# Russoul/cuda-mat

Hardware: AMD Instinct MI355X
Metric: BiCGSTAB iters/sec + SpMV effective HBM GB/s, 10M-row CSR at 1/2/4/8 GPUs (higher is better)
Workload: dtype f64

## Files before the change

### cuda_mat_amd/csrc/device.h

```cpp
#pragma once
#include <hip/hip_runtime.h>

#include "batch.h"
#include "kernels.h"
#include "steps.h"

namespace cm {

__device__ __forceinline__ double wave_sum(double v)
{
#pragma unroll
    for (int o = 32; o > 0; o >>= 1) v += __shfl_xor(v, o, 64);
    return v;
}

template <int L>
__device__ __forceinline__ double group_sum(double v)
{
#pragma unroll
    for (int o = L / 2; o > 0; o >>= 1) v += __shfl_xor(v, o, 64);
    return v;
}

template <int K>
__device__ __forceinline__ void block_sum(double (&v)[K], double *lds)
{
    const int wave = threadIdx.x >> 6, lane = threadIdx.x & 63;
#pragma unroll
    for (int k = 0; k < K; k++) v[k] = wave_sum(v[k]);
    __syncthreads();
    if (lane == 0) {
#pragma unroll
        for (int k = 0; k < K; k++) lds[wave * K + k] = v[k];
    }
    __syncthreads();
#pragma unroll
    for (int k = 0; k < K; k++)
        v[k] = ((lds[0 * K + k] + lds[1 * K + k]) + lds[2 * K + k]) + lds[3 * K + k];
}

constexpr int kLongRow = 4096;
constexpr int kLongRowSlots = 32;

struct LongRows {
    int rows[kLongRowSlots];
    int noted;
    int count;
    int next;
};

__device__ __forceinline__ void long_rows_note(LongRows &t, int row)
{
    const int slot = atomicAdd(&t.noted, 1);
    if (slot < kLongRowSlots) t.rows[slot] = row;
}

__device__ __forceinline__ int long_rows_round(LongRows &t, const int *rp, int row_begin, int row_end, int done)
{
    const int total = t.noted;
    if (done >= total) return 0;
    if (threadIdx.x == 0) {
        if (total <= kLongRowSlots) {
            for (int i = 1; i < total; i++) {
                const int r = t.rows[i];
                int j = i - 1;
                while (j >= 0 && t.rows[j] > r) { t.rows[j + 1] = t.rows[j]; j--; }
                t.rows[j + 1] = r;
            }
            t.count = total;
        } else {
            int r = done == 0 ? row_begin : t.next, m = 0;
            for (; r < row_end && m < kLongRowSlots; r++)
                if (rp[r + 1] - rp[r] > kLongRow) t.rows[m++] = r;
            t.count = m;
            t.next = r;
        }
    }
    __syncthreads();
    return t.count;
}

template <int K>
__device__ __forceinline__ void load_scalars(const ScalarSrc &s, double (&out)[K], double *lds)
{
    if (s.count == 0) {
#pragma unroll
        for (int k = 0; k < K; k++) out[k] = s.ptr[k];
        return;
    }
#pragma unroll
    for (int k = 0; k < K; k++) out[k] = 0.0;
    for (int j = threadIdx.x; j < s.count; j += kBlock) {
#pragma unroll
        for (int k = 0; k < K; k++) out[k] += s.ptr[(size_t)j * s.stride + k];
    }
    block_sum<K>(out, lds);
}

__device__ __forceinline__ bool leader() { return blockIdx.x == 0 && threadIdx.x == 0; }

__device__ __forceinline__ int uniform_state(const LoopState *st)
{
    __shared__ int s_state;
    if (threadIdx.x == 0) s_state = st->state;
    __syncthreads();
    const int v = s_state;
    __syncthreads();
    return v;
}

__device__ __forceinline__ void publish_progress(const LoopArgs &la, int state)
{
    if (la.snap && leader())
        __hip_atomic_store(&la.snap[la.k % la.snap_slots],
                           ((unsigned long long)(unsigned)(la.k + 1) << 32) | (unsigned long long)(unsigned)state,
                           __ATOMIC_RELAXED, __HIP_MEMORY_SCOPE_SYSTEM);
}

constexpr double kTolabsMin = 0x1p-485;

__device__ __forceinline__ bool init_refusal(double nrm0, double tolabs, bool r_nonzero)
{
    return !isfinite(nrm0) || (nrm0 == 0.0 && r_nonzero) || (tolabs > 0.0 && tolabs < kTolabsMin);
}

__device__ __forceinline__ bool check_half(const LoopArgs &la, const ScalarSrc &half, double *lds)
{
    LoopState *st = la.st;
    if (uniform_state(st) != 0) return true;
    double sc[1];
    load_scalars<1>(half, sc, lds);
    const double nrm = sqrt(sc[0]);
    const int it = st->it;
    if (la.loop == CUDAMAT_LOOP_PBICGSTAB) {
        if (leader()) {
            st->nrm = nrm;
            if (la.hist && 2 * it < la.hist_cap) la.hist[2 * it] = nrm;
        }
        if (!la.no_exit && nrm < st->tolabs) {
            if (leader()) st->state = 1;
            return true;
        }
        if (!la.no_exit && isnan(nrm)) {
            if (leader()) st->state = 3;
            return true;
        }
    }
    return false;
}

__device__ __forceinline__ bool check_full(const LoopArgs &la, const double (&sc)[2])
{
    LoopState *st = la.st;
    const int it = st->it;
    if (it == 0) return false;
    const double nrm = sqrt(sc[1]);
    const double omega = st->omega;
    if (leader()) {
        st->nrm = nrm;
        if (la.hist) {
            const int slot = (la.loop != CUDAMAT_LOOP_PBICGSTAB2) ? 2 * (it - 1) + 1 : it - 1;
            if (slot < la.hist_cap) la.hist[slot] = nrm;
        }
    }
    if (la.no_exit) return false;
    if (nrm < st->tolabs) {
        if (leader()) st->state = 2;
        return true;
    }
    if (la.loop == CUDAMAT_LOOP_PBICGSTAB2 && (fabs(omega) < 1e-5 || isnan(omega))) {
        if (leader()) st->state = 3;
        return true;
    }
    if (isnan(nrm)) {
        if (leader()) st->state = 3;
        return true;
    }
    return false;
}

template <int K>
__device__ __forceinline__ void load_row(const double *p, int64_t i, double (&v)[K])
{
    if constexpr (K == 1) {
        v[0] = p[i];
    } else {
        const double2 *q = (const double2 *)(p + (size_t)i * K);
#pragma unroll
        for (int h = 0; h < K / 2; h++) {
            const double2 t = q[h];
            v[2 * h] = t.x;
            v[2 * h + 1] = t.y;
        }
    }
}

template <int K>
__device__ __forceinline__ void store_row(double *p, int64_t i, const double (&v)[K], unsigned mask)
{
    if constexpr (K == 1) {
        if (mask & 1u) p[i] = v[0];
    } else {
        double *row = p + (size_t)i * K;
#pragma unroll
        for (int h = 0; h < K / 2; h++) {
            const unsigned m = (mask >> (2 * h)) & 3u;
            if (m == 3u) ((double2 *)row)[h] = make_double2(v[2 * h], v[2 * h + 1]);
            else if (m == 1u) row[2 * h] = v[2 * h];
            else if (m == 2u) row[2 * h + 1] = v[2 * h + 1];
        }
    }
}

constexpr unsigned kAll = 0xffu;
// ... 143 lines not shown
```

### cuda_mat_amd/csrc/loops.hip

```cpp
#include <utility>
#include <math.h>
#include <stdlib.h>
#include <string.h>

#include "solver.h"

using namespace cm;

namespace cm {

int wait_progress(cudamat_solver *s, hipStream_t st, int j, const char *what, unsigned long long *word)
{
    volatile unsigned long long *slot = &s->snap_host[j % kRing];
    unsigned long long w = *slot;
    if ((unsigned)(w >> 32) != (unsigned)(j + 1)) {
        const double t_wait = now_s();
        while ((unsigned)((w = *slot) >> 32) != (unsigned)(j + 1)) {
            __builtin_ia32_pause();
            if (now_s() - t_wait > 30.0) {
                const double t_drain = now_s();
                while (hipStreamQuery(st) == hipErrorNotReady && now_s() - t_drain < 5.0) __builtin_ia32_pause();
                set_error("%siteration %d did not report progress within 30 s%s", what, j,
                          s->sharded ? " (sharded run: this rank must exit, its peers are waiting in a collective)" : "");
                return CUDAMAT_ERR_HIP;
// ... 67 lines not shown
    int pipe_rr = kPipeRR;
    ScalarSrc pipeB_src{nullptr, 0, 1};
    hipStream_t rst = nullptr;

    void prof_mark() { if (profile && hipEventRecord(prof_event(s, pe++), st) != hipSuccess) s->prof_failed = true; }

    int setup();
    int pipelined_prologue();
    bool wants_fused() const;
    bool wants_resident();
    int run_resident(bool *gave_up);
    int run_host_loop();
    int iterate_reference();
    int iterate_fused();
    int iterate_pipelined(int k);
    int pipe_reduce(ScalarSrc parts, int K, double *out, int slot);
    int pipe_wait(int slot);
    int finish(bool *precond_gave_up, cudamat_stats *out);
};

int Solve::setup()
{
    CM_ARG(s && b && x, "null pointer");
    CM_ARG(precond == CUDAMAT_PRECOND_NONE || precond == CUDAMAT_PRECOND_ILU0 || precond == CUDAMAT_PRECOND_BLOCK_ILU0,
           "precond");
    CM_ARG(loop == CUDAMAT_LOOP_PBICGSTAB || loop == CUDAMAT_LOOP_PBICGSTAB2 || loop == CUDAMAT_LOOP_PIPELINED, "loop");
    CM_ARG(maxit >= 0, "maxit");
    CM_ARG(!(precond == CUDAMAT_PRECOND_ILU0 && s->sharded),
           "ILU(0) of the whole matrix is single-GPU only (SURVEY 8e); sharded runs take CUDAMAT_PRECOND_BLOCK_ILU0");
    CM_ARG(!(precond && s->d), "the (A0 + I d) variant has no preconditioner (pbicgstab.h:110)");
    CM_HIP(hipSetDevice(s->ctx->device));
    cfg = &s->ctx->cfg;
    t_begin = now_s();
    st = s->ctx->stream;
    n = s->n;
    x_user = x;
    {
        int rc_setup = ensure_work(s);
        const bool defer_form = s->spmv_mode < 0 && precond == CUDAMAT_PRECOND_ILU0 && !s->sharded;
        if (rc_setup == CUDAMAT_OK && !defer_form) rc_setup = ensure_spmv_mode(s);
        if (rc_setup == CUDAMAT_OK && precond && (!s->has_ilu || (s->sharded && !s->ilu_block)))
            rc_setup = ilu0_setup(s, precond == CUDAMAT_PRECOND_BLOCK_ILU0);
        CM_TRY(setup_agree(s, rc_setup));
    }
    perm = precond == CUDAMAT_PRECOND_ILU0 && !s->sharded && loop == CUDAMAT_LOOP_PBICGSTAB && s->L.lm && s->U.lm && !s->d &&
           cfg->trsv_perm && !s->perm_failed;
    if (perm && !s->perm_ready) {
        const int rcp = ilu_perm_matrix(s);
        if (rcp == CUDAMAT_ERR_NOMEM) { perm = false; s->perm_failed = true; }
        else CM_TRY(rcp);
    }
    s->perm_active = perm;
    if (!perm && s->spmv_mode < 0) CM_TRY(ensure_spmv_mode(s));
    if (perm) {
        CM_TRY(perm_to_space(s, false, b, s->b_perm));
        if (!(flags & CUDAMAT_FLAG_X0_ONES)) CM_TRY(perm_to_space(s, true, x, s->x_perm));
        b = s->b_perm;
        x = s->x_perm;
    }

    const int need_hist = history_need(loop, maxit);
    hist_base = abs_tol > 0.0 ? (s->hist_count < s->hist_cap ? s->hist_count : s->hist_cap) : 0;
    if (hist_base == 0 && need_hist > s->hist_cap) {
        if (s->hist) { CM_HIP(hipStreamSynchronize(st)); CM_DROP(hipFree(s->hist)); s->hist = nullptr; }
        CM_TRY(dev_alloc((void **)&s->hist, sizeof(double) * (size_t)need_hist));
        s->hist_cap = need_hist;
    }
    if (s->hist_cap > hist_base)
        CM_HIP(hipMemsetAsync(s->hist + hist_base, 0xFF, sizeof(double) * (size_t)(s->hist_cap - hist_base), st));
    s->last_loop = loop;
    profile = (flags & CUDAMAT_FLAG_PROFILE) != 0;
    sharded = s->sharded;
    pipelined = loop == CUDAMAT_LOOP_PIPELINED;
    pipe_pc = pipelined && precond != CUDAMAT_PRECOND_NONE;
    la = LoopArgs{s->st, s->hist + hist_base, s->hist_cap - hist_base, loop, (flags & CUDAMAT_FLAG_NO_EXIT) ? 1 : 0, s->snap_dev, kRing, 0};
    for (int i = 0; i < kRing; i++) s->snap_host[i] = 0ULL;

    s->comm_used = 0;
    s->comm_kind.clear();
    s->profiling = profile && sharded;
    s->prof_failed = false;
    t_loop0 = now_s();
    if (flags & CUDAMAT_FLAG_X0_ONES) CM_TRY(launch_fill(st, n, 1.0, x));
    CM_HIP(hipMemcpyAsync(s->pw, x, sizeof(double) * (size_t)n, hipMemcpyDeviceToDevice, st));
    CM_TRY(spmv_local(s, s->pw, s->r, 0, nullptr, nullptr, la_none, CHECK_NONE, nosrc));
    CM_TRY(launch_init(st, n, b, s->r, s->rw, s->p, s->parts_full, &np_full));
    full_src = ScalarSrc{s->parts_full, np_full, 2};
    if (sharded) {
        CM_TRY(launch_reduce_parts(st, full_src, 2, s->red + 4, 0));
        CM_TRY(allreduce(s, s->red + 4, 2));
        full_src = ScalarSrc{s->red + 4, 0, 1};
    }
    CM_TRY(launch_init_finish(st, s->st, full_src, tol, abs_tol, la.no_exit, sharded ? nullptr : s->r, n));
    return CUDAMAT_OK;
}

int Solve::pipelined_prologue()
{
    pipe_rr = cfg->pipe_rr >= 0 ? cfg->pipe_rr : kPipeRR;
    const size_t nb = sizeof(double) * (size_t)(s->n_pad > 0 ? s->n_pad : 1);
    if (!s->pz) {
        double **vs[] = {&s->pz, &s->pww, &s->pq, &s->py, &s->pxh};
        for (double **q : vs) {
            CM_TRY(dev_alloc((void **)q, nb));
            CM_HIP(hipMemsetAsync(*q, 0, nb, st));
        }
        CM_TRY(dev_alloc((void **)&s->pipeA, sizeof(double) * 3 * kVecGridMax));
        CM_TRY(dev_alloc((void **)&s->pipeB, sizeof(double) * 5 * kVecGridMax));
        CM_TRY(dev_alloc((void **)&s->red_pipe, sizeof(double) * 16));
    }
    if (pipe_pc && !s->prh) {
        double **vs[] = {&s->prh, &s->pwh, &s->psh, &s->pzh, &s->pqh, &s->ptmp};
        for (double **q : vs) {
            CM_TRY(dev_alloc((void **)q, nb));
            CM_HIP(hipMemsetAsync(*q, 0, nb, st));
        }
    }
    if (sharded && s->comm.allreduce_side && s->comm.reduce_stream) {
        rst = (hipStream_t)s->comm.reduce_stream;
        for (int e = 0; e < 2; e++) {
            if (!s->ev_red[e]) CM_HIP(hipEventCreateWithFlags(&s->ev_red[e], hipEventDisableTiming));
            if (!s->ev_red_done[e]) CM_HIP(hipEventCreateWithFlags(&s->ev_red_done[e], hipEventDisableTiming));
        }
    }
    const LoopArgs la_freeze{s->st, nullptr, 0, loop, 0};
    const double *rh0 = s->r;
    if (pipe_pc) { CM_TRY(precond_apply(s, s->r, s->ptmp, s->prh)); rh0 = s->prh; }
    CM_TRY(spmv_local(s, rh0, s->pww, 1, s->rw, s->parts_rv, la_freeze, CHECK_NONE, nosrc));
    ScalarSrc rww{s->parts_rv, spmv_parts(s), 2};
    if (sharded) {
        CM_TRY(launch_reduce_parts(st, rww, 1, s->red + 0, 0));
        CM_TRY(allreduce(s, s->red + 0, 1));
        rww = ScalarSrc{s->red + 0, 0, 1};
    }
    const double *wh0 = s->pww;
    if (pipe_pc) { CM_TRY(precond_apply(s, s->pww, s->ptmp, s->pwh)); wh0 = s->pwh; }
    CM_TRY(spmv_local(s, wh0, s->t, 0, nullptr, nullptr, la_freeze, CHECK_NONE, nosrc));
    CM_TRY(launch_pipe_seed(st, full_src, rww, s->red_pipe + 8));
    pipeB_src = ScalarSrc{s->red_pipe + 8, 0, 1};
    return CUDAMAT_OK;
}

int Solve::pipe_reduce(ScalarSrc parts, int K, double *out, int slot)
{
    if (!sharded) return CUDAMAT_OK;
    if (rst) {
        CM_HIP(hipEventRecord(s->ev_red[slot], st));
        CM_HIP(hipStreamWaitEvent(rst, s->ev_red[slot], 0));
        CM_TRY(launch_reduce_parts(rst, parts, K, out, 0));
        comm_mark_begin(s, 3, rst);
        if (s->comm.allreduce_side(s->comm.user, out, K) != 0) { set_error("allreduce_side callback failed"); return CUDAMAT_ERR_COMM; }
        comm_mark_end(s, rst);
        CM_HIP(hipEventRecord(s->ev_red_done[slot], rst));
    } else {
        CM_TRY(launch_reduce_parts(st, parts, K, out, 0));
        CM_TRY(allreduce(s, out, K));
    }
    return CUDAMAT_OK;
}

int Solve::pipe_wait(int slot)
{
    if (sharded && rst) CM_HIP(hipStreamWaitEvent(st, s->ev_red_done[slot], 0));
    return CUDAMAT_OK;
}

int Solve::iterate_pipelined(int k)
{
// ... 431 lines not shown
```

### cuda_mat_amd/csrc/solver.h

```cpp
#pragma once
#include <vector>

#include "kernels.h"
#include "spmv_pb.h"
#include "valdict.h"
#include "spmv_sell.h"
#include "spmv_pat.h"

namespace cm {

constexpr int kLag = 2;
constexpr int kRing = kLag + 2;
constexpr int kPipeRR = 32;

struct TriFactor {
    int nlevels = 0;
    std::vector<int> level_ptr;
    int *rp = nullptr;
    int *ci = nullptr;
    double *val = nullptr;
    int *row_of = nullptr;
    double *dinv = nullptr;
    int64_t nnz = 0;
    int *rhs_of = nullptr, *out_of = nullptr;
// ... 47 lines not shown
    double *v2 = nullptr;
    double *pz = nullptr, *pww = nullptr, *pq = nullptr, *py = nullptr, *pxh = nullptr;
    double *prh = nullptr, *pwh = nullptr, *psh = nullptr, *pzh = nullptr, *pqh = nullptr, *ptmp = nullptr;
    double *pipeA = nullptr, *pipeB = nullptr, *red_pipe = nullptr;
    hipEvent_t ev_red[2] = {}, ev_red_done[2] = {};

    double *parts_full = nullptr, *parts_rv = nullptr, *parts_half = nullptr, *parts_tt = nullptr;
    double *red = nullptr;
    cm::LoopState *st = nullptr;
    cm::LoopState *st_ring = nullptr;
    hipEvent_t ev[cm::kRing] = {};
    unsigned long long *snap_host = nullptr;
    unsigned long long *snap_dev = nullptr;
    double *hist = nullptr;
    int hist_cap = 0;
    int hist_count = 0;
    int last_loop = 0;

    std::vector<hipEvent_t> prof_ev;
    std::vector<hipEvent_t> comm_ev;
    std::vector<int> comm_kind;
    size_t comm_used = 0;
    bool profiling = false;
    bool prof_failed = false;

    bool sharded = false;
    cudamat_comm comm{};
    bool overlap = false;
    bool agreed = false;
    int overlap_chunks = 4;
    hipEvent_t ev_x = nullptr, ev_part[cm::kPbMaxChunks] = {};
    hipStream_t part_stream[cm::kPbMaxChunks] = {};
    hipEvent_t ev_p1[cm::kPbMaxChunks] = {};
    double ms_spmv_alone = 0.0;
    bool windowed = false;
    bool windows_known = false;
    std::vector<int64_t> w_send_off, w_send_cnt, w_recv_off, w_recv_cnt;
    double gather_fraction = 1.0;
    double *need_dev = nullptr;

    bool has_ilu = false;
    int *pm_rp = nullptr, *pm_ci = nullptr;
    double *pm_val = nullptr;
    int64_t pm_nnz = 0;
    bool pm_owned = false;
    bool ilu_block = false;
    double *lu = nullptr;
    int *diag_pos = nullptr;
    cm::TriFactor L, U;
    void *ilu_plans = nullptr;
    cm::PbPlan pb_perm{};
    cm::ValDict vd_perm;
    double *x_perm = nullptr, *b_perm = nullptr;
    bool perm_ready = false;
    bool perm_failed = false;
    bool perm_active = false;
    double t_perm_matrix = 0.0;
    double t_analysis = 0.0, t_factor = 0.0, t_analysis_l = 0.0, t_analysis_u = 0.0;
    int trsv_fallbacks = 0;
    cm::ValDict vd;
    bool vd_tried = false;
    unsigned *bar = nullptr;
    int test_allreduces = 0;
    bool resident_off = false;
    int device_cus = 0;
    int loop_fallbacks = 0;

    cm::ManyWork many;
};

namespace cm {
int dev_alloc(void **p, size_t bytes);
int solver_alloc(cudamat_ctx *ctx, int n_local, int64_t n_cols, int64_t nnz, cudamat_solver **out);
int solver_setup_pattern(cudamat_solver *s);
int solver_setup_values(cudamat_solver *s);
int spmv_mode_is_blocked_early(cudamat_solver *s, bool *blocked);
void spmv_mode_adopt_blocked(cudamat_solver *s, const PbPlan &pb, double seconds);
int ensure_valdict(cudamat_solver *s);
int ensure_work(cudamat_solver *s);
int ensure_spmv_mode(cudamat_solver *s);
int setup_agree(cudamat_solver *s, int rc_local);
int spmv_local(cudamat_solver *s, const double *x_local, double *y, int dot, const double *w, double *parts, LoopArgs la, int check,
               ScalarSrc half);
int spmv_parts(const cudamat_solver *s);
int allreduce(cudamat_solver *s, double *buf, int count);
void comm_mark_begin(cudamat_solver *s, int kind, hipStream_t st);
void comm_mark_end(cudamat_solver *s, hipStream_t st);
hipEvent_t prof_event(cudamat_solver *s, size_t i);
int precond_apply(cudamat_solver *s, const double *in, double *tmp, double *out, bool native = false);

constexpr int kSortRowMax = 1024;
int launch_sort_rows(hipStream_t st, int nrows, const int *src_rp, const int *src_of, const int *dst_rp, const int *ci,
                     const double *val, const int *colmap, int *out_ci, double *out_val);
int ilu0_setup(cudamat_solver *s, bool block);
int ilu0_analyse_early(cudamat_solver *s);
void ilu0_flush_deferred(cudamat_solver *s);
bool ilu0_will_use_level_major(cudamat_solver *s);
int ilu0_release(cudamat_solver *s);
int trsv_apply(cudamat_solver *s, const TriFactor &F, bool upper, const double *rhs, double *out);
int precond_apply_original(cudamat_solver *s, const double *in, double *tmp, double *out);
int perm_to_space(cudamat_solver *s, bool upper, const double *in, double *out);
int perm_from_space(cudamat_solver *s, bool upper, const double *in, double *out);
int ilu_perm_matrix(cudamat_solver *s);
int trsv_status(cudamat_solver *s);
bool trsv_syncfree_active(cudamat_solver *s);
int trsv_form_code(cudamat_solver *s);
void trsv_group_counts(cudamat_solver *s, int *groups_l, int *groups_u);
void trsv_disable_syncfree(cudamat_solver *s);
void many_release(cudamat_solver *s);
int wait_progress(cudamat_solver *s, hipStream_t st, int j, const char *what, unsigned long long *word);
int history_need(int loop, int maxit);
int history_count(int loop, const LoopState &f, int cap);
void stats_from_state(const LoopState &f, cudamat_stats *o);
void stats_ilu0(cudamat_solver *s, bool applied, cudamat_stats *o);
}
```

### cuda_mat_amd/csrc/solver.hip

```cpp
#include <mutex>
#include <utility>
#include <math.h>
#include <stdlib.h>
#include <string.h>

#include "solver.h"

using namespace cm;

namespace cm {

int dev_alloc(void **p, size_t bytes)
{
    *p = nullptr;
    hipError_t e = hipMalloc(p, bytes ? bytes : 16);
    if (e != hipSuccess) {
        set_error("hipMalloc(%zu bytes) failed: %s", bytes, hipGetErrorString(e));
        return e == hipErrorOutOfMemory ? CUDAMAT_ERR_NOMEM : CUDAMAT_ERR_HIP;
    }
    return CUDAMAT_OK;
}

static void free_work(cudamat_solver *s)
{
// ... 230 lines not shown
        if (e) CM_DROP(hipEventDestroy(e));
    for (hipStream_t q : s->part_stream)
        if (q) { CM_DROP(hipStreamSynchronize(q)); CM_DROP(hipStreamDestroy(q)); }
    delete s;
    return CUDAMAT_OK;
}

extern "C" int cudamat_solver_set_shift(cudamat_solver *s, const double *d)
{
    CM_ARG(s, "solver is NULL");
    s->d = d;
    return CUDAMAT_OK;
}

extern "C" int cudamat_solver_set_comm(cudamat_solver *s, const cudamat_comm *comm)
{
    CM_ARG(s, "solver is NULL");
    CM_HIP(hipStreamSynchronize(s->ctx->stream));
    free_work(s);
    pb_free(&s->pb);
    sell_free(&s->sell);
    pat_free(&s->pat);
    ilu0_release(s);
    s->spmv_mode = -1;
    s->overlap = false;
    s->agreed = false;
    s->windowed = false;
    s->windows_known = false;
    if (s->need_dev) { CM_DROP(hipFree(s->need_dev)); s->need_dev = nullptr; }
    const bool forced = comm && comm->world == 1 && s->ctx->cfg.force_sharded;
    if (!comm || (comm->world <= 1 && !forced)) {
        s->sharded = false;
        s->n_pad = s->n;
        return CUDAMAT_OK;
    }
    CM_ARG(comm->allgather && comm->allreduce, "collectives missing");
    CM_ARG(comm->rank >= 0 && comm->rank < comm->world, "rank");
    const int64_t per = (s->n_cols + comm->world - 1) / comm->world;
    int64_t mine = s->n_cols - per * comm->rank;
    if (mine > per) mine = per;
    if (mine < 0) mine = 0;
    if (mine != s->n) {
        set_error("row block mismatch: rank %d of %d must own %lld rows of %lld (uniform blocks of %lld), has %d",
                  comm->rank, comm->world, (long long)mine, (long long)s->n_cols, (long long)per, s->n);
        return CUDAMAT_ERR_ARG;
    }
    s->comm = *comm;
    s->sharded = true;
    s->n_pad = (int)per;
    if (comm->gather_window && comm->world > 1 && comm->world <= 4096)
        CM_TRY(dev_alloc((void **)&s->need_dev, sizeof(double) * ((size_t)2 * comm->world + (size_t)2 * comm->world * comm->world)));
    if (comm->gather_part && comm->comm_stream && !s->ev_x) {
        CM_HIP(hipEventCreateWithFlags(&s->ev_x, hipEventDisableTiming));
        for (int c = 0; c < kPbMaxChunks; c++) {
            CM_HIP(hipEventCreateWithFlags(&s->ev_part[c], hipEventDisableTiming));
            CM_HIP(hipEventCreateWithFlags(&s->ev_p1[c], hipEventDisableTiming));
            CM_HIP(hipStreamCreateWithFlags(&s->part_stream[c], hipStreamNonBlocking));
        }
    }
    if (s->ctx->cfg.overlap_chunks >= 1 && s->ctx->cfg.overlap_chunks <= kPbMaxChunks) s->overlap_chunks = s->ctx->cfg.overlap_chunks;
    return CUDAMAT_OK;
}

namespace cm {

static hipEvent_t comm_event(cudamat_solver *s)
{
    if (s->comm_used == s->comm_ev.size()) {
        hipEvent_t e = nullptr;
        if (hipEventCreate(&e) != hipSuccess) s->prof_failed = true;
        s->comm_ev.push_back(e);
    }
    return s->comm_ev[s->comm_used++];
}
void comm_mark_begin(cudamat_solver *s, int kind, hipStream_t st)
{
    if (!s->profiling) return;
    s->comm_kind.push_back(kind);
    if (hipEventRecord(comm_event(s), st) != hipSuccess) s->prof_failed = true;
}
void comm_mark_end(cudamat_solver *s, hipStream_t st)
{
    if (s->profiling && hipEventRecord(comm_event(s), st) != hipSuccess) s->prof_failed = true;
}

int spmv_local(cudamat_solver *s, const double *x_local, double *y, int dot, const double *w,
               double *parts, LoopArgs la, int check, ScalarSrc half)
{
    Range range_spmv(s->sharded ? "cudamat: SpMV + exchange of its input" : "cudamat: SpMV");
    const double *xfull = x_local;
    const bool windowed = s->sharded && s->windowed;
    const bool overlapped = s->sharded && !windowed && s->overlap && s->spmv_mode == 1;
    if (windowed) {
        hipStream_t st = s->ctx->stream;
        CM_HIP(hipMemcpyAsync(s->gather + (size_t)s->comm.rank * (size_t)s->n_pad, x_local, sizeof(double) * (size_t)s->n_pad,
                              hipMemcpyDeviceToDevice, st));
        comm_mark_begin(s, 2, st);
        if (s->comm.gather_window(s->comm.user, x_local, s->gather, (int64_t)s->n_pad, s->w_send_off.data(), s->w_send_cnt.data(),
                                  s->w_recv_off.data(), s->w_recv_cnt.data()) != 0) {
            set_error("gather_window callback failed");
            return CUDAMAT_ERR_COMM;
        }
        comm_mark_end(s, st);
    } else if (s->sharded && !overlapped) {
        comm_mark_begin(s, 2, s->ctx->stream);
        if (s->comm.allgather(s->comm.user, x_local, s->gather, (int64_t)s->n_pad) != 0) {
            set_error("allgather callback failed");
            return CUDAMAT_ERR_COMM;
        }
        comm_mark_end(s, s->ctx->stream);
    }
    if (s->sharded) xfull = s->gather;
    SpmvArgs a{};
    a.n = s->n;
    a.rp = s->rp;
    a.ci = s->ci;
    a.val = s->val;
    a.x = xfull;
    a.d = s->d;
    a.xd = x_local;
    a.alpha = 1.0;
    a.beta = 0.0;
    a.y = y;
    a.dot = dot;
    a.w = w;
    a.parts = parts;
    a.loop = la;
    a.check = check;
    a.half = half;
    a.pb_strict = 0;
    if (s->spmv_mode == 1 || s->perm_active) CM_TRY(pb_strict_for(s->ctx, &a.pb_strict));
    if (overlapped) {
        hipStream_t st = s->ctx->stream, cst = (hipStream_t)s->comm.comm_stream;
        const PbPlan &p = s->pb;
        CM_HIP(hipEventRecord(s->ev_x, st));
        CM_HIP(hipStreamWaitEvent(cst, s->ev_x, 0));
        comm_mark_begin(s, 0, cst);
        for (int c = 0; c < p.chunks; c++) {
            const int64_t off = (int64_t)c * p.chunk_len;
            int64_t cnt = (int64_t)s->n_pad - off;
            if (cnt > p.chunk_len) cnt = p.chunk_len;
            if (cnt > 0 && s->comm.gather_part(s->comm.user, x_local, s->gather, (int64_t)s->n_pad, off, cnt) != 0) {
                set_error("gather_part callback failed");
                return CUDAMAT_ERR_COMM;
            }
            CM_HIP(hipEventRecord(s->ev_part[c], cst));
        }
        comm_mark_end(s, cst);
        CM_HIP(hipMemcpyAsync(s->gather + (size_t)s->comm.rank * (size_t)s->n_pad, x_local, sizeof(double) * (size_t)s->n_pad,
                              hipMemcpyDeviceToDevice, st));
        CM_TRY(launch_pb_check(st, a));
        CM_TRY(launch_pb_phase1(st, p, a, 0));
        for (int c = 0; c < p.chunks; c++) {
            hipStream_t ps = s->part_stream[c];
            CM_HIP(hipStreamWaitEvent(ps, s->ev_x, 0));
            CM_HIP(hipStreamWaitEvent(ps, s->ev_part[c], 0));
            CM_TRY(launch_pb_phase1(ps, p, a, 1 + c));
            CM_HIP(hipEventRecord(s->ev_p1[c], ps));
        }
        for (int c = 0; c < p.chunks; c++) CM_HIP(hipStreamWaitEvent(st, s->ev_p1[c], 0));
        return launch_pb_phase2(st, p, a);
    }
    if (s->perm_active) return launch_spmv_pb(s->ctx->stream, s->pb_perm, a);
    if (s->spmv_mode == 1) return launch_spmv_pb(s->ctx->stream, s->pb, a);
    if (s->spmv_mode == 2) return launch_spmv_sell(s->ctx->stream, s->sell, a);
    if (s->spmv_mode == 3) return launch_spmv_pat(s->ctx->stream, s->pat, a);
// ... 448 lines not shown
```

### cuda_mat_amd/csrc/spmv_pb.h

```cpp
#pragma once
#include "kernels.h"
#include "valdict.h"

namespace cm {

constexpr int kPbMaxChunks = 16;

struct PbCols {
    int64_t per = 0;
    int chunks = 1;
    int rank = 0;
};

struct PbPlan {
    int n = 0;
    int64_t n_cols = 0;
    int64_t nnz = 0;
    int CB = 0, NCB = 0;
    int64_t per = 0;
    int chunks = 1;
    int64_t chunk_len = 0;
    int bpc = 0;
    int RB = 0, NRB = 0;
    int NW = 0;
    int SR = 0;
    int LPS = 64;
    int depth = 4;
    int NSUB = 0;
    double *pv = nullptr;
    unsigned char *pvi = nullptr;
    const double *dict = nullptr;
    int ndict = 0;
    unsigned short *pc = nullptr;
    unsigned short *pr = nullptr;
    double *P = nullptr;
    int *cstart = nullptr;
    int *col0 = nullptr;
    int *sstart = nullptr;
    int *slen = nullptr;
    int *order = nullptr;
    int part_off[kPbMaxChunks + 2] = {0};
    int placed = -1;
    int place_slabs = 0;
    double place_seconds = 0.0;
    float place_check_ms = 0.f, place_fast_ms = 0.f, place_slow_ms = 0.f;
    char place_classes[192] = {0};
    bool pc_zeroed = false;
    double build_seconds = 0.0;
};

struct PbCut {
    int per, chunks, chunk_len, bpc, CB;
};
struct PbBuild {
    PbPlan p;
    int *bins = nullptr;
    PbCut cut{};
    size_t cap = 0;
    double t0 = 0.0;
    bool verbose = false;
    bool two_pass = false;
    int place = 0;
    bool report_classes = false;
    double place_max_seconds = 0.3;
    int fill_occ = 0;
    int GB = 1, NG = 1;
    unsigned long long *smeta = nullptr;
    int *gstart = nullptr;
};
int pb_build_begin(hipStream_t st, const Config &cfg, int n, int64_t n_cols, int64_t nnz, const int *rp, const int *ci,
                   const PbCols *cols, PbBuild *b);
int pb_build_alloc(hipStream_t st, const Config &cfg, int n, int64_t n_cols, int64_t nnz, const PbCols *cols, PbBuild *b);
int pb_build_count(hipStream_t st, const Config &cfg, const int *rp, const int *ci, PbBuild *b);
int pb_build_values(hipStream_t st, PbBuild *b, const ValDict *vd);
int pb_build_fill(hipStream_t st, PbBuild *b, const int *rp, const int *ci, const double *val, const ValDict *vd, int sub0, int sub1);
int pb_build_end(hipStream_t st, PbBuild *b, PbPlan *out);
void pb_build_abort(PbBuild *b);

bool pb_candidate(hipStream_t st, int n, int64_t n_cols, int64_t nnz, const int *rp, const int *ci);
int pb_build(hipStream_t st, const Config &cfg, int n, int64_t n_cols, int64_t nnz, const int *rp, const int *ci,
             const double *val, PbPlan *out, const PbCols *cols = nullptr, const ValDict *vd = nullptr);
void pb_free(PbPlan *p);
int pb_strict_for(cudamat_ctx *ctx, int *strict);
int launch_spmv_pb(hipStream_t st, const PbPlan &plan, const SpmvArgs &a);
int launch_pb_check(hipStream_t st, const SpmvArgs &a);
int launch_pb_phase1(hipStream_t st, const PbPlan &plan, const SpmvArgs &a, int part);
int launch_pb_phase2(hipStream_t st, const PbPlan &plan, const SpmvArgs &a);

}
```

### cuda_mat_amd/csrc/spmv_pb.hip

```cpp
#include <algorithm>
#include <map>
#include <mutex>
#include <string>
#include <vector>

#include "spmv_pb.h"

namespace cm {

typedef unsigned short u16;
constexpr int kPbBuildWaves = 4;
constexpr int kP1Threads = 1024;
constexpr int kP1Unroll = 8;
constexpr int kTileMax = 13312;
constexpr int kPbAlign = 64;

template <typename T>
static int dalloc(T **p, size_t count)
{
    *p = nullptr;
    hipError_t e = hipMalloc((void **)p, sizeof(T) * (count ? count : 1));
    if (e != hipSuccess) {
        set_error("hipMalloc(%zu bytes) failed: %s", sizeof(T) * count, hipGetErrorString(e));
        return e == hipErrorOutOfMemory ? CUDAMAT_ERR_NOMEM : CUDAMAT_ERR_HIP;
    }
    return CUDAMAT_OK;
}

void pb_free(PbPlan *p)
{
    void *ptrs[] = {p->pv, p->pvi, p->pc, p->pr, p->P, p->cstart, p->col0, p->sstart, p->slen, p->order};
    for (void *q : ptrs)
        if (q) CM_DROP(hipFree(q));
    *p = PbPlan();
}

bool pb_candidate(hipStream_t st, int n, int64_t n_cols, int64_t nnz, const int *rp, const int *ci)
{
    (void)st; (void)rp; (void)ci;
    if (n < 65536 || nnz < (1 << 20) || n_cols * 8 < (1 << 20)) return false;
    if ((double)nnz / n < 4.0) return false;
    if ((int64_t)n > (int64_t)kMaxParts * kTileMax) return false;
    return true;
}

__device__ __forceinline__ int col_to_cb(const PbCut &c, int col)
{
    const int q = col / c.per, w = col - q * c.per;
    const int ch = w / c.chunk_len, off = w - ch * c.chunk_len;
    return (q * c.chunks + ch) * c.bpc + off / c.CB;
}

__device__ __forceinline__ int col_to_cb_fast(const PbCut &c, double inv_cb, int col)
{
    if (c.chunks == 1 && col < c.per) {
        int cb = (int)((double)col * inv_cb);
        cb -= (long long)cb * c.CB > (long long)col ? 1 : 0;
        cb += (long long)(cb + 1) * c.CB <= (long long)col ? 1 : 0;
        return cb;
    }
    return col_to_cb(c, col);
}

__device__ __forceinline__ int wave_match_rank(unsigned long long *tab, int key, bool active, int lane, int nkeys, int *count_of_key_lane)
{
    if (lane < nkeys) tab[lane] = 0ULL;
    __builtin_amdgcn_fence(__ATOMIC_RELEASE, "wavefront");
    __builtin_amdgcn_wave_barrier();
    if (active) atomicOr(&tab[key], 1ULL << lane);
    __builtin_amdgcn_fence(__ATOMIC_RELEASE, "wavefront");
    __builtin_amdgcn_wave_barrier();
    const unsigned long long mine = active ? tab[key] : 0ULL;
    *count_of_key_lane = lane < nkeys ? __popcll(tab[lane]) : 0;
    __builtin_amdgcn_fence(__ATOMIC_RELEASE, "wavefront");
    __builtin_amdgcn_wave_barrier();
    return __popcll(mine & ((1ULL << lane) - 1ULL));
}

template <bool FILL>
__global__ __launch_bounds__(64 * kPbBuildWaves) void k_pb_rows(int n, const int *rp, const int *ci,
                                                               const double *val, PbCut cut, const int *col0, int NCB,
                                                               int SR, int NSUB, int *bins, double *pv, u16 *pc, u16 *pr,
                                                               const unsigned char *vidx, unsigned char *pvi, int sub0, int sub1)
{
    extern __shared__ int lds_i[];
    const int wave = threadIdx.x >> 6, lane = threadIdx.x & 63;
    const int sub = sub0 + blockIdx.x * kPbBuildWaves + wave;
    if (sub >= sub1) return;
// ... 841 lines not shown
    for (int v : hl) {
        hist[v == 0 ? 0 : v <= 8 ? 1 : v <= 24 ? 2 : v <= 48 ? 3 : v <= 64 ? 4 : v <= 128 ? 5 : 6]++;
        if (v > 64) in_long += v;
    }
    fprintf(stderr, "[cudamat] pb arrays: pv %p pvi %p pc %p pr %p P %p sstart %p slen %p cstart %p\n", (void *)p.pv, (void *)p.pvi, (void *)p.pc,
            (void *)p.pr, (void *)p.P, (void *)p.sstart, (void *)p.slen, (void *)p.cstart);
    fprintf(stderr, "[cudamat] pb plan: %d x %lld, nnz %lld, NCB %d (CB %d), NSUB %d (NW %d, SR %d), LPS %d, depth %d; segments: "
                    "empty %lld, 1-8 %lld, 9-24 %lld, 25-48 %lld, 49-64 %lld, 65-128 %lld, >128 %lld; %.1f %% of the entries in "
                    "segments longer than a wave\n",
            p.n, (long long)p.n_cols, (long long)p.nnz, p.NCB, p.CB, p.NSUB, p.NW, p.SR, p.LPS, p.depth, hist[0], hist[1], hist[2], hist[3],
            hist[4], hist[5], hist[6], 100.0 * (double)in_long / (double)(p.nnz > 0 ? p.nnz : 1));
}

static void place_report_classes(hipStream_t st, const PbPlan &p, size_t cap)
{
    if (!pool_enabled()) return;
    PlaceTimer tm(st);
    if (!tm.ok) return;
    int dev = 0;
    if (hipGetDevice(&dev) != hipSuccess) return;
    std::lock_guard<std::mutex> lock(g_place_mu);
    PlaceMemo &m = g_place[dev];
    if (m.gen != pool_generation()) { m.gen = pool_generation(); m.reset(); }
    std::vector<char *> slabs;
    std::vector<char *> scratch(3, nullptr);
    for (int k = 0; k < 4 && !(scratch[0] && scratch[1] && scratch[2]); k++) {
        char *base = nullptr;
        if (hipMalloc(&base, kPlaceSlab) != hipSuccess) { CM_DROP(hipGetLastError()); break; }
        slabs.push_back(base);
        char *seg = nullptr;
        size_t bytes = 0;
        if (!pool_segment_of(base, &seg, &bytes)) break;
        char *b0 = seg + ((size_t)(base - seg) + kPlaceBlock - 1) / kPlaceBlock * kPlaceBlock;
        for (char *q = b0; q + kPlaceBlock <= base + bytes; q += kPlaceBlock) {
            const int c = place_class_of(tm, m, q);
            if (c >= 0 && c < 3 && !scratch[c]) scratch[c] = q;
        }
    }
    struct Arr { const char *name; const char *ptr; size_t bytes; };
    const Arr arrs[4] = {{"values", p.pv ? (const char *)p.pv : (const char *)p.pvi, p.pv ? sizeof(double) * cap : cap},
                         {"col idx", (const char *)p.pc, sizeof(u16) * cap}, {"row idx", (const char *)p.pr, sizeof(u16) * cap}, {"products", (const char *)p.P, sizeof(double) * cap}};
    for (const Arr &a : arrs) {
        std::string line;
        for (size_t off = 0; off + kPlaceSample <= a.bytes; off += kPlaceSample) {
            int cls = -1;
            float worst = 0.f;
            for (int k = 0; k < 3; k++) {
                if (!scratch[k]) continue;
                const float t = tm.ms(a.ptr + off, scratch[k] + kPlaceBlock - kPlaceSample, kPlaceSample);
                if (t > worst) { worst = t; cls = k; }
            }
            line += cls < 0 || !(m.t_hi >= kPlaceGap * m.t_lo) || worst <= sqrtf(m.t_lo * m.t_hi) ? '?' : (char)('0' + cls);
        }
        fprintf(stderr, "[cudamat] pb classes: %-8s at %p, per %zu MB: %s\n", a.name, (const void *)a.ptr, kPlaceSample >> 20, line.c_str());
    }
    for (char *q : slabs) CM_DROP(hipFree(q));
}

int pb_build_end(hipStream_t st, PbBuild *b, PbPlan *out)
{
    if (hipStreamSynchronize(st) != hipSuccess) { set_error("pb fill failed"); pb_build_abort(b); return CUDAMAT_ERR_HIP; }
    if (b->verbose) pb_print_plan(b->p);
    if (b->report_classes && sizeof(double) * b->cap >= kPlaceMinBytes) place_report_classes(st, b->p, b->cap);
    pb_scratch_free(b);
    CM_DROP(hipFree(b->bins));
    b->bins = nullptr;
    b->p.build_seconds = now_s() - b->t0;
    *out = b->p;
    b->p = PbPlan();
    return CUDAMAT_OK;
}

int pb_build(hipStream_t st, const Config &cfg, int n, int64_t n_cols, int64_t nnz, const int *rp, const int *ci,
             const double *val, PbPlan *out, const PbCols *cols, const ValDict *vd)
{
    PbBuild b;
    CM_TRY(pb_build_begin(st, cfg, n, n_cols, nnz, rp, ci, cols, &b));
    CM_TRY(pb_build_values(st, &b, vd));
    CM_TRY(pb_build_fill(st, &b, rp, ci, val, vd, 0, b.p.NSUB));
    return pb_build_end(st, &b, out);
}


__global__ __launch_bounds__(kP1Threads) void k_pb_phase1(const double *x, const int *col0, const int *list,
                                                          const int *cstart, const double *pv, const u16 *pc,
                                                          double *P, const LoopState *st, int cb0)
{
    extern __shared__ __attribute__((aligned(16))) double xs[];
    if (st && st->state != 0) return;
    const int cb = list ? list[blockIdx.x] : (int)blockIdx.x + cb0;
    const int s = cstart[cb], e = cstart[cb + 1];
    if (s >= e) return;
    const int c0 = col0[cb], cn = col0[cb + 1] - c0;
    for (int i = threadIdx.x; i < cn; i += kP1Threads) xs[i] = x[c0 + i];
    __syncthreads();
    constexpr int STEP = 2 * kP1Threads;
    const int k0 = (s & ~1) + 2 * (int)threadIdx.x;
    for (int k = k0; k < e; k += 4 * STEP) {
        double2 v[4];
        ushort2 c[4];
        bool full[4];
#pragma unroll
        for (int u = 0; u < 4; u++) {
            const int kk = k + u * STEP;
            full[u] = kk >= s && kk + 1 < e;
            if (full[u]) {
                v[u] = *(const double2 *)(pv + kk);
                c[u] = *(const ushort2 *)(pc + kk);
            }
        }
#pragma unroll
        for (int u = 0; u < 4; u++) {
            const int kk = k + u * STEP;
            if (full[u]) {
                double2 o;
                o.x = v[u].x * xs[c[u].x];
                o.y = v[u].y * xs[c[u].y];
                *(double2 *)(P + kk) = o;
            } else {
                if (kk >= s && kk < e) P[kk] = pv[kk] * xs[pc[kk]];
                if (kk + 1 >= s && kk + 1 < e) P[kk + 1] = pv[kk + 1] * xs[pc[kk + 1]];
            }
        }
    }
}

__global__ __launch_bounds__(kP1Threads) void k_pb_phase1_dict(const double *x, const int *col0, const int *list,
                                                               const int *cstart, const unsigned char *pvi, const u16 *pc,
                                                               const double *dict, int cb_doubles, double *P,
                                                               const LoopState *st, int cb0)
{
    extern __shared__ __attribute__((aligned(16))) double xs[];
    if (st && st->state != 0) return;
    const int cb = list ? list[blockIdx.x] : (int)blockIdx.x + cb0;
    const int s = cstart[cb], e = cstart[cb + 1];
    if (s == e) return;
    double *dv = xs + cb_doubles;
    const int c0 = col0[cb], cn = col0[cb + 1] - c0;
    for (int i = threadIdx.x; i < cn; i += kP1Threads) xs[i] = x[c0 + i];
    if (threadIdx.x < kDictMax) dv[threadIdx.x] = dict[threadIdx.x];
    __syncthreads();
    constexpr int U = kP1Unroll, STEP = 2 * kP1Threads, CH = U * STEP;
    const int a0 = (s + 1) & ~1;
    if (threadIdx.x == 0 && s < a0) P[s] = dv[pvi[s]] * xs[pc[s]];
    int kb = a0;
    const int t2 = 2 * (int)threadIdx.x;
    for (; kb + CH <= e; kb += CH) {
        const int k = kb + t2;
        u16 iv[U];
        unsigned cv[U];
#pragma unroll
        for (int u = 0; u < U; u++) {
            iv[u] = *(const u16 *)(pvi + k + u * STEP);
            cv[u] = *(const unsigned *)(pc + k + u * STEP);
        }
#pragma unroll
        for (int u = 0; u < U; u++) {
            double2 o;
            o.x = dv[iv[u] & 0xffu] * xs[cv[u] & 0xffffu];
            o.y = dv[iv[u] >> 8] * xs[cv[u] >> 16];
            *(double2 *)(P + k + u * STEP) = o;
        }
    }
    {
        const int m = e > kb ? (e - kb) / STEP : 0;
        const int k = kb + t2;
        u16 iv[U - 1];
        unsigned cv[U - 1];
#pragma unroll
        for (int u = 0; u < U - 1; u++) {
            if (u < m) {
                iv[u] = *(const u16 *)(pvi + k + u * STEP);
                cv[u] = *(const unsigned *)(pc + k + u * STEP);
            }
        }
#pragma unroll
        for (int u = 0; u < U - 1; u++) {
            if (u < m) {
                double2 o;
                o.x = dv[iv[u] & 0xffu] * xs[cv[u] & 0xffffu];
                o.y = dv[iv[u] >> 8] * xs[cv[u] >> 16];
                *(double2 *)(P + k + u * STEP) = o;
            }
        }
        const int kr = k + m * STEP;
        if (kr + 1 < e) {
            const u16 iw = *(const u16 *)(pvi + kr);
            const unsigned cw = *(const unsigned *)(pc + kr);
            double2 o;
            o.x = dv[iw & 0xffu] * xs[cw & 0xffffu];
            o.y = dv[iw >> 8] * xs[cw >> 16];
            *(double2 *)(P + kr) = o;
        } else if (kr < e) {
            P[kr] = dv[pvi[kr]] * xs[pc[kr]];
        }
    }
}

struct Pb2Args {
    int n, NCB, SR;
    const int *sstart, *slen;
    const double *P;
    const u16 *pr;
    const double *d, *xd;
    double alpha, beta;
    double *y;
    int dot;
    const double *w;
    double *parts;
    const LoopState *st;
    int strict;
};

__device__ __forceinline__ void pb_seg_add(double *my, int r, double p, bool on, int lane, int group_first, bool strict)
{
    if (!strict) {
// ... 125 lines not shown
            const int g = lane / LPS, li = lane % LPS;
            for (int j = 0; j < lim; j += DEPTH * G) {
                int s[DEPTH], l[DEPTH];
                double pv4[DEPTH];
                int r4[DEPTH];
#pragma unroll
                for (int u = 0; u < DEPTH; u++) {
                    const int cbi = j + u * G + g;
                    s[u] = __shfl(mys, cbi & 63, 64);
                    l[u] = cbi < 64 ? __shfl(myl, cbi & 63, 64) : 0;
                }
#pragma unroll
                for (int u = 0; u < DEPTH; u++) {
                    const bool on = li < l[u];
                    pv4[u] = on ? a.P[s[u] + li] : 0.0;
                    r4[u] = on ? (int)a.pr[s[u] + li] : 0;
                }
#pragma unroll
                for (int u = 0; u < DEPTH; u++) {
                    if (!a.strict) {
                        if (li < l[u]) unsafeAtomicAdd(&my[r4[u]], pv4[u]);
                    } else {
#pragma unroll
                        for (int gg = 0; gg < G; gg++)
                            pb_seg_add(my, r4[u], pv4[u], g == gg && li < l[u], lane, gg * LPS, true);
                    }
                }
            }
        }
    }
    __builtin_amdgcn_fence(__ATOMIC_RELEASE, "wavefront");
    __builtin_amdgcn_wave_barrier();
    double acc0 = 0.0, acc1 = 0.0;
    const long long row0 = (long long)sub * a.SR;
    for (int i = lane; i < a.SR && row0 + i < a.n; i += 64) {
#pragma clang fp contract(off)
        const int row = (int)(row0 + i);
        double sum = my[i];
        if (a.d) {
            const double dx = a.d[row] * a.xd[row];
            sum = sum + dx;
        }
        double out = a.alpha * sum;
        if (a.beta != 0.0) {
            const double by = a.beta * a.y[row];
            out = out + by;
        }
        a.y[row] = out;
        if (a.dot) {
            acc0 += out * a.w[row];
            acc1 += out * out;
        }
    }
    if (a.dot) {
        double *red = yt + (size_t)NW * a.SR;
#pragma unroll
        for (int o = 32; o > 0; o >>= 1) {
            acc0 += __shfl_xor(acc0, o, 64);
            acc1 += __shfl_xor(acc1, o, 64);
        }
        if (lane == 0) {
            red[2 * wave] = acc0;
            red[2 * wave + 1] = acc1;
        }
        __syncthreads();
        if (threadIdx.x == 0) {
            double t0 = 0.0, t1 = 0.0;
            for (int q = 0; q < NW; q++) {
                t0 += red[2 * q];
                t1 += red[2 * q + 1];
            }
            a.parts[2 * blockIdx.x] = t0;
            a.parts[2 * blockIdx.x + 1] = t1;
        }
    }
}

int launch_pb_check(hipStream_t st, const SpmvArgs &a)
{
    if (a.loop.st && a.check == CHECK_HALF) CM_TRY(launch_check(st, a.loop, a.half, CHECK_HALF));
    return CUDAMAT_OK;
}

static int launch_pb_phase1_blocks(hipStream_t st, const PbPlan &p, const SpmvArgs &a, const int *list, int first, int last)
{
    if (last <= first) return CUDAMAT_OK;
    if (p.pvi) {
        CM_TRY(set_max_lds((const void *)k_pb_phase1_dict));
        const int cbd = (p.CB + 1) & ~1;
        hipLaunchKernelGGL(k_pb_phase1_dict, dim3(last - first), dim3(kP1Threads), sizeof(double) * (size_t)(cbd + kDictMax), st, a.x,
                           p.col0, list ? list + first : (const int *)nullptr, p.cstart, p.pvi, p.pc, p.dict, cbd, p.P, a.loop.st,
                           list ? 0 : first);
        CM_HIP(hipGetLastError());
        return CUDAMAT_OK;
    }
    CM_TRY(set_max_lds((const void *)k_pb_phase1));
    hipLaunchKernelGGL(k_pb_phase1, dim3(last - first), dim3(kP1Threads), sizeof(double) * (size_t)p.CB, st, a.x, p.col0,
                       list ? list + first : (const int *)nullptr, p.cstart, p.pv, p.pc, p.P, a.loop.st, list ? 0 : first);
    CM_HIP(hipGetLastError());
    return CUDAMAT_OK;
}

int launch_pb_phase1(hipStream_t st, const PbPlan &p, const SpmvArgs &a, int part)
{
    if (part < 0) return launch_pb_phase1_blocks(st, p, a, nullptr, 0, p.NCB);
    return launch_pb_phase1_blocks(st, p, a, p.order, p.part_off[part], p.part_off[part + 1]);
}

int launch_spmv_pb(hipStream_t st, const PbPlan &p, const SpmvArgs &a)
{
    CM_TRY(launch_pb_check(st, a));
    CM_TRY(launch_pb_phase1(st, p, a, -1));
    return launch_pb_phase2(st, p, a);
}

int launch_pb_phase2(hipStream_t st, const PbPlan &p, const SpmvArgs &a)
{
    Pb2Args b;
    b.n = p.n; b.NCB = p.NCB; b.SR = p.SR;
    b.sstart = p.sstart; b.slen = p.slen;
    b.P = p.P; b.pr = p.pr;
    b.d = a.d; b.xd = a.xd;
    b.alpha = a.alpha; b.beta = a.beta;
    b.y = a.y; b.dot = a.dot; b.w = a.w; b.parts = a.parts;
    b.st = a.loop.st;
    b.strict = a.pb_strict;
    const size_t lds = sizeof(double) * ((size_t)p.NW * p.SR + 2 * (size_t)p.NW);
#define CM_P2D(NWV, LPSV, DV)                                                                             \
    do {                                                                                                  \
        CM_TRY(set_max_lds((const void *)k_pb_phase2<NWV, LPSV, DV>));                                   \
        hipLaunchKernelGGL((k_pb_phase2<NWV, LPSV, DV>), dim3(p.NRB), dim3(64 * NWV), lds, st, b);       \
    } while (0)
#define CM_P2(NWV, LPSV)                                                                                  \
    do {                                                                                                  \
        if (p.depth >= 16) CM_P2D(NWV, LPSV, 16);                                                         \
        else if (p.depth >= 8) CM_P2D(NWV, LPSV, 8);                                                      \
        else CM_P2D(NWV, LPSV, 4);                                                                        \
    } while (0)
#define CM_P2_LPS(NWV)                                           \
    do {                                                         \
        if (p.LPS == 16) CM_P2(NWV, 16);                         \
        else if (p.LPS == 32) CM_P2(NWV, 32);                    \
        else CM_P2(NWV, 64);                                     \
    } while (0)
    switch (p.NW) {
    case 4:  CM_P2_LPS(4); break;
    case 8:  CM_P2_LPS(8); break;
    default: CM_P2_LPS(16); break;
    }
#undef CM_P2_LPS
#undef CM_P2
#undef CM_P2D
    CM_HIP(hipGetLastError());
    return CUDAMAT_OK;
}

}
```

Before: 184.1.

## Fuse half-step residual check into SpMV phase1 and skip phase1 for ones start vector

```diff
diff --git a/cuda_mat_amd/csrc/device.h b/cuda_mat_amd/csrc/device.h
--- a/cuda_mat_amd/csrc/device.h
+++ b/cuda_mat_amd/csrc/device.h
@@ -22,14 +22,14 @@
     return v;
 }
 
-template <int K>
+template <int K, int W = kBlock>
 __device__ __forceinline__ void block_sum(double (&v)[K], double *lds)
 {
     const int wave = threadIdx.x >> 6, lane = threadIdx.x & 63;
 #pragma unroll
     for (int k = 0; k < K; k++) v[k] = wave_sum(v[k]);
     __syncthreads();
-    if (lane == 0) {
+    if (lane == 0 && (W == kBlock || wave < kBlock / 64)) {
 #pragma unroll
         for (int k = 0; k < K; k++) lds[wave * K + k] = v[k];
     }
@@ -80,7 +80,7 @@
     return t.count;
 }
 
-template <int K>
+template <int K, int W = kBlock>
 __device__ __forceinline__ void load_scalars(const ScalarSrc &s, double (&out)[K], double *lds)
 {
     if (s.count == 0) {
@@ -90,11 +90,13 @@
     }
 #pragma unroll
     for (int k = 0; k < K; k++) out[k] = 0.0;
-    for (int j = threadIdx.x; j < s.count; j += kBlock) {
-#pragma unroll
-        for (int k = 0; k < K; k++) out[k] += s.ptr[(size_t)j * s.stride + k];
-    }
-    block_sum<K>(out, lds);
+    if (W == kBlock || threadIdx.x < kBlock) {
+        for (int j = threadIdx.x; j < s.count; j += kBlock) {
+#pragma unroll
+            for (int k = 0; k < K; k++) out[k] += s.ptr[(size_t)j * s.stride + k];
+        }
+    }
+    block_sum<K, W>(out, lds);
 }
 
 __device__ __forceinline__ bool leader() { return blockIdx.x == 0 && threadIdx.x == 0; }
@@ -124,12 +126,13 @@
     return !isfinite(nrm0) || (nrm0 == 0.0 && r_nonzero) || (tolabs > 0.0 && tolabs < kTolabsMin);
 }
 
+template <int W = kBlock>
 __device__ __forceinline__ bool check_half(const LoopArgs &la, const ScalarSrc &half, double *lds)
 {
     LoopState *st = la.st;
     if (uniform_state(st) != 0) return true;
     double sc[1];
-    load_scalars<1>(half, sc, lds);
+    load_scalars<1, W>(half, sc, lds);
     const double nrm = sqrt(sc[0]);
     const int it = st->it;
     if (la.loop == CUDAMAT_LOOP_PBICGSTAB) {
diff --git a/cuda_mat_amd/csrc/loops.hip b/cuda_mat_amd/csrc/loops.hip
--- a/cuda_mat_amd/csrc/loops.hip
+++ b/cuda_mat_amd/csrc/loops.hip
@@ -173,8 +173,12 @@
     s->prof_failed = false;
     t_loop0 = now_s();
     if (flags & CUDAMAT_FLAG_X0_ONES) CM_TRY(launch_fill(st, n, 1.0, x));
-    CM_HIP(hipMemcpyAsync(s->pw, x, sizeof(double) * (size_t)n, hipMemcpyDeviceToDevice, st));
-    CM_TRY(spmv_local(s, s->pw, s->r, 0, nullptr, nullptr, la_none, CHECK_NONE, nosrc));
+    if ((flags & CUDAMAT_FLAG_X0_ONES) && spmv_ones_shortcut(s)) {
+        CM_TRY(spmv_local_ones(s, s->r));
+    } else {
+        CM_HIP(hipMemcpyAsync(s->pw, x, sizeof(double) * (size_t)n, hipMemcpyDeviceToDevice, st));
+        CM_TRY(spmv_local(s, s->pw, s->r, 0, nullptr, nullptr, la_none, CHECK_NONE, nosrc));
+    }
     CM_TRY(launch_init(st, n, b, s->r, s->rw, s->p, s->parts_full, &np_full));
     full_src = ScalarSrc{s->parts_full, np_full, 2};
     if (sharded) {
diff --git a/cuda_mat_amd/csrc/solver.h b/cuda_mat_amd/csrc/solver.h
--- a/cuda_mat_amd/csrc/solver.h
+++ b/cuda_mat_amd/csrc/solver.h
@@ -153,6 +153,8 @@
 int setup_agree(cudamat_solver *s, int rc_local);
 int spmv_local(cudamat_solver *s, const double *x_local, double *y, int dot, const double *w, double *parts, LoopArgs la, int check,
                ScalarSrc half);
+bool spmv_ones_shortcut(const cudamat_solver *s);
+int spmv_local_ones(cudamat_solver *s, double *y);
 int spmv_parts(const cudamat_solver *s);
 int allreduce(cudamat_solver *s, double *buf, int count);
 void comm_mark_begin(cudamat_solver *s, int kind, hipStream_t st);
diff --git a/cuda_mat_amd/csrc/solver.hip b/cuda_mat_amd/csrc/solver.hip
--- a/cuda_mat_amd/csrc/solver.hip
+++ b/cuda_mat_amd/csrc/solver.hip
@@ -336,6 +336,32 @@
 void comm_mark_end(cudamat_solver *s, hipStream_t st)
 {
     if (s->profiling && hipEventRecord(comm_event(s), st) != hipSuccess) s->prof_failed = true;
+}
+
+static const PbPlan *blocked_whole(const cudamat_solver *s)
+{
+    if (s->sharded) return nullptr;
+    if (s->perm_active) return &s->pb_perm;
+    return s->spmv_mode == 1 ? &s->pb : nullptr;
+}
+
+bool spmv_ones_shortcut(const cudamat_solver *s)
+{
+    const PbPlan *p = blocked_whole(s);
+    return p && p->pv && !s->d;
+}
+
+int spmv_local_ones(cudamat_solver *s, double *y)
+{
+    Range range_spmv("cudamat: SpMV");
+    SpmvArgs a{};
+    a.n = s->n;
+    a.alpha = 1.0;
+    a.beta = 0.0;
+    a.y = y;
+    a.check = CHECK_NONE;
+    CM_TRY(pb_strict_for(s->ctx, &a.pb_strict));
+    return launch_spmv_pb_ones(s->ctx->stream, *blocked_whole(s), a);
 }
 
 int spmv_local(cudamat_solver *s, const double *x_local, double *y, int dot, const double *w,
diff --git a/cuda_mat_amd/csrc/spmv_pb.h b/cuda_mat_amd/csrc/spmv_pb.h
--- a/cuda_mat_amd/csrc/spmv_pb.h
+++ b/cuda_mat_amd/csrc/spmv_pb.h
@@ -83,8 +83,9 @@
 void pb_free(PbPlan *p);
 int pb_strict_for(cudamat_ctx *ctx, int *strict);
 int launch_spmv_pb(hipStream_t st, const PbPlan &plan, const SpmvArgs &a);
+int launch_spmv_pb_ones(hipStream_t st, const PbPlan &plan, const SpmvArgs &a);
 int launch_pb_check(hipStream_t st, const SpmvArgs &a);
 int launch_pb_phase1(hipStream_t st, const PbPlan &plan, const SpmvArgs &a, int part);
-int launch_pb_phase2(hipStream_t st, const PbPlan &plan, const SpmvArgs &a);
+int launch_pb_phase2(hipStream_t st, const PbPlan &plan, const SpmvArgs &a, const double *products = nullptr);
 
 }
diff --git a/cuda_mat_amd/csrc/spmv_pb.hip b/cuda_mat_amd/csrc/spmv_pb.hip
--- a/cuda_mat_amd/csrc/spmv_pb.hip
+++ b/cuda_mat_amd/csrc/spmv_pb.hip
@@ -4,6 +4,7 @@
 #include <string>
 #include <vector>
 
+#include "device.h"
 #include "spmv_pb.h"
 
 namespace cm {
@@ -1011,12 +1012,22 @@
 }
 
 
+__device__ __forceinline__ bool pb_phase1_enter(const LoopArgs &la, int check, const ScalarSrc &half)
+{
+    if (!la.st) return false;
+    if (check == CHECK_HALF && blockIdx.x == 0) {
+        __shared__ double lds[8];
+        return check_half<kP1Threads>(la, half, lds);
+    }
+    return la.st->state != 0;
+}
+
 __global__ __launch_bounds__(kP1Threads) void k_pb_phase1(const double *x, const int *col0, const int *list,
                                                           const int *cstart, const double *pv, const u16 *pc,
-                                                          double *P, const LoopState *st, int cb0)
+                                                          double *P, LoopArgs la, int check, ScalarSrc half, int cb0)
 {
     extern __shared__ __attribute__((aligned(16))) double xs[];
-    if (st && st->state != 0) return;
+    if (pb_phase1_enter(la, check, half)) return;
     const int cb = list ? list[blockIdx.x] : (int)blockIdx.x + cb0;
     const int s = cstart[cb], e = cstart[cb + 1];
     if (s >= e) return;
@@ -1057,10 +1068,10 @@
 __global__ __launch_bounds__(kP1Threads) void k_pb_phase1_dict(const double *x, const int *col0, const int *list,
                                                                const int *cstart, const unsigned char *pvi, const u16 *pc,
                                                                const double *dict, int cb_doubles, double *P,
-                                                               const LoopState *st, int cb0)
+                                                               LoopArgs la, int check, ScalarSrc half, int cb0)
 {
     extern __shared__ __attribute__((aligned(16))) double xs[];
-    if (st && st->state != 0) return;
+    if (pb_phase1_enter(la, check, half)) return;
     const int cb = list ? list[blockIdx.x] : (int)blockIdx.x + cb0;
     const int s = cstart[cb], e = cstart[cb + 1];
     if (s == e) return;
@@ -1352,21 +1363,22 @@
     return CUDAMAT_OK;
 }
 
-static int launch_pb_phase1_blocks(hipStream_t st, const PbPlan &p, const SpmvArgs &a, const int *list, int first, int last)
-{
-    if (last <= first) return CUDAMAT_OK;
+static int launch_pb_phase1_blocks(hipStream_t st, const PbPlan &p, const SpmvArgs &a, const int *list, int first, int last,
+                                   int check = CHECK_NONE)
+{
+    if (last <= first) return check == CHECK_HALF ? launch_pb_check(st, a) : CUDAMAT_OK;
     if (p.pvi) {
         CM_TRY(set_max_lds((const void *)k_pb_phase1_dict));
         const int cbd = (p.CB + 1) & ~1;
         hipLaunchKernelGGL(k_pb_phase1_dict, dim3(last - first), dim3(kP1Threads), sizeof(double) * (size_t)(cbd + kDictMax), st, a.x,
-                           p.col0, list ? list + first : (const int *)nullptr, p.cstart, p.pvi, p.pc, p.dict, cbd, p.P, a.loop.st,
-                           list ? 0 : first);
+                           p.col0, list ? list + first : (const int *)nullptr, p.cstart, p.pvi, p.pc, p.dict, cbd, p.P, a.loop, check,
+                           a.half, list ? 0 : first);
         CM_HIP(hipGetLastError());
         return CUDAMAT_OK;
     }
     CM_TRY(set_max_lds((const void *)k_pb_phase1));
     hipLaunchKernelGGL(k_pb_phase1, dim3(last - first), dim3(kP1Threads), sizeof(double) * (size_t)p.CB, st, a.x, p.col0,
-                       list ? list + first : (const int *)nullptr, p.cstart, p.pv, p.pc, p.P, a.loop.st, list ? 0 : first);
+                       list ? list + first : (const int *)nullptr, p.cstart, p.pv, p.pc, p.P, a.loop, check, a.half, list ? 0 : first);
     CM_HIP(hipGetLastError());
     return CUDAMAT_OK;
 }
@@ -1379,17 +1391,23 @@
 
 int launch_spmv_pb(hipStream_t st, const PbPlan &p, const SpmvArgs &a)
 {
-    CM_TRY(launch_pb_check(st, a));
-    CM_TRY(launch_pb_phase1(st, p, a, -1));
+    const int check = a.loop.st && a.check == CHECK_HALF ? CHECK_HALF : CHECK_NONE;
+    CM_TRY(launch_pb_phase1_blocks(st, p, a, nullptr, 0, p.NCB, check));
     return launch_pb_phase2(st, p, a);
 }
 
-int launch_pb_phase2(hipStream_t st, const PbPlan &p, const SpmvArgs &a)
+int launch_spmv_pb_ones(hipStream_t st, const PbPlan &p, const SpmvArgs &a)
+{
+    if (!p.pv || a.d) { set_error("launch_spmv_pb_ones: needs fp64 values and no shift"); return CUDAMAT_ERR_ARG; }
+    return launch_pb_phase2(st, p, a, p.pv);
+}
+
+int launch_pb_phase2(hipStream_t st, const PbPlan &p, const SpmvArgs &a, const double *products)
 {
     Pb2Args b;
     b.n = p.n; b.NCB = p.NCB; b.SR = p.SR;
     b.sstart = p.sstart; b.slen = p.slen;
-    b.P = p.P; b.pr = p.pr;
+    b.P = products ? products : p.P; b.pr = p.pr;
     b.d = a.d; b.xd = a.xd;
     b.alpha = a.alpha; b.beta = a.beta;
     b.y = a.y; b.dot = a.dot; b.w = a.w; b.parts = a.parts;
```

New measurement: 185.4 (median of 6 runs). About the same (+0.7%).
